# DefaultRui/VLN-VER

Measured on AMD Instinct MI355X. Metric: viewpoints/sec (multi-view->voxel fwd+bwd), vocc.py config, higher is better.
Workload: dtype bf16

## Files before the change

scratch/lattice_mfma_shape_ab.py:

```python
import argparse
import importlib
import json
import os
import shutil
import statistics
import sys
import tempfile

import torch

ROOT = os.path.dirname(os.path.dirname(os.path.abspath(__file__)))
sys.path.insert(0, ROOT)
hip = importlib.import_module('vln-ver_amd.hipops')
ups = importlib.import_module('vln-ver_amd.dense_heads.upsample')


def load(path):
    hip._lib, hip.LIB_PATH = None, os.path.abspath(path)
    return hip.lib()


def timed(f, n=5):
    f()
    torch.cuda.synchronize()
    a, b = torch.cuda.Event(enable_timing=True), torch.cuda.Event(enable_timing=True)
    a.record()
    for _ in range(n):
        f()
    b.record()
    torch.cuda.synchronize()
    return a.elapsed_time(b) / n


def main():
    ap = argparse.ArgumentParser()
    ap.add_argument('arms', nargs='+', help='name=path; the first is the parent')
    ap.add_argument('--reps', type=int, default=5)
    ap.add_argument('--out', default=None)
    args = ap.parse_args()
    arms = [a.split('=', 1) for a in args.arms]
    tmp = tempfile.mkdtemp()
    arms.append(['parent_copy', shutil.copy(arms[0][1], os.path.join(tmp, 'libver_hip_parent_copy.so'))])
    handles = [(name, load(path)) for name, path in arms]
    out = open(args.out, 'a') if args.out else None

    def emit(rec):
        line = json.dumps(rec)
        print(line, flush=True)
        if out:
            out.write(line + '\n')
            out.flush()

    B, DEV, C, N, layout, hc = 192, 'cuda', 768, 1536, 3, 30
    plan = ups._layer_plan_z4(C, torch.device(DEV))[0]
    m = B * 2 * hc * hc
    e = torch.randn(4, B, 2, hc // 2, hc // 2, 2, C, device=DEV).bfloat16()
    table, _ = ups._const_rows_z4(C, hc, hc, torch.device(DEV), torch.bfloat16)
    g = torch.randn(m, N, device=DEV).bfloat16()
    cls = [(ups._class_segments_z4(c, C), plan[c][1] - plan[c][0]) for c in ups._CLASSES]
    ws = [torch.randn(k, N, device=DEV).bfloat16() for _, k in cls]
    dws = [torch.empty(k, N, dtype=torch.bfloat16, device=DEV) for _, k in cls]
    y = torch.empty(m, N, dtype=torch.bfloat16, device=DEV)
    flops = 2.0 * m * N * sum(k for _, k in cls)

    def forward():
        for (segs, _), w in zip(cls, ws):
            hip.gemm_nn_taps(e, layout, (hc, hc), segs, w, const_rows=table, out=y)

    def wgrad():
        for (segs, _), dw in zip(cls, dws):
            hip.wgrad_tn_segments(e, layout, (hc, hc), segs, g, out=dw, const_rows=table)

    for fam, f in (('gemm_nn_segments', forward), ('wgrad_tn_segments', wgrad)):
        samples = {name: [] for name, _ in handles}
        for _ in range(args.reps):
            for name, h in handles:
                hip._lib = h
                samples[name].append(timed(f))
        med = {k: statistics.median(v) for k, v in samples.items()}
        spread = abs(med[arms[0][0]] - med['parent_copy'])
        for name, _ in handles:
            emit(dict(kind='microbench', family=fam, operands='N(0,1)', arm=name, M=m, K=sum(k for _, k in cls), N=N,
                      ms=[round(x, 4) for x in samples[name]], ms_median=round(med[name], 4), tflops=round(flops / med[name] / 1e9, 1)))
        for name, _ in handles[1:-1]:
            gain = med[arms[0][0]] - med[name]
            emit(dict(kind='verdict', family=fam, operands='N(0,1)', arm=name, parent_ms=round(med[arms[0][0]], 4), new_ms=round(med[name], 4),
                      parent_aa_spread_ms=round(spread, 4), gain_ms=round(gain, 4), speedup=round(med[arms[0][0]] / med[name], 4),
                      clears_twice_the_spread=bool(gain > 2 * spread)))
    shutil.rmtree(tmp, ignore_errors=True)


if __name__ == '__main__':
    main()
```

vln-ver_amd/csrc/ver_gemm.hip:

```cpp
#include "ver_common.h"

namespace {
typedef __bf16 bf16x8 __attribute__((ext_vector_type(8)));
typedef float f32x16 __attribute__((ext_vector_type(16)));
typedef int i32x2 __attribute__((ext_vector_type(2)));
typedef int i32x4 __attribute__((ext_vector_type(4)));
typedef __attribute__((address_space(3))) void lds_void;

constexpr int kTile = 256;
constexpr int kStageBytes = 32768;
constexpr int kStages = 4;
constexpr int kLdsBytes = kStages * kStageBytes;

template <int OFF>
__device__ __forceinline__ i32x2 tr_read(int addr) {
    i32x2 v;
    asm volatile("ds_read_b64_tr_b16 %0, %1 offset:%2" : "=v"(v) : "v"(addr), "n"(OFF) : "memory");
    return v;
}
template <int OFF>
__device__ __forceinline__ i32x4 row_read(int addr) {
    i32x4 v;
    asm volatile("ds_read_b128 %0, %1 offset:%2" : "=v"(v) : "v"(addr), "n"(OFF) : "memory");
    return v;
}
__device__ __forceinline__ bf16x8 frag(i32x2 lo, i32x2 hi) {
    return __builtin_bit_cast(bf16x8, (i32x4)__builtin_shufflevector(lo, hi, 0, 1, 2, 3));
}

struct TapArgs {
    const __bf16* lattice;
    long lattice_bytes;
    int B, H, W, C, ntaps, P;
    const float* rowpos;
    const __bf16* cst;
    long cst_bytes;
    int CW, ncst;
    signed char kind[64], dz[64], dy[64], dx[64];
    signed char pl[64];
    long plane_elems;
};

struct GemmArgs {
    const __bf16* A;
    const __bf16* W;
    const float* bias;
    __bf16* C;
    long lda, ldw, ldc, M;
    int K, N, tiles_n, T, per_xcd;
    int S, Kc;
    float* ws;
    TapArgs t;
};

struct GemmLane {
    int offA0, offA1;
    int offB0, offB1;
    int voA, voW;
    int stepW;
    int stepA16;
    int dmaA, dmaW;
};

constexpr int kOutside = (int)0x80000000;
template <int L>
__device__ __forceinline__ int cell_off(const TapArgs& t, int b, int zl, int y, int x, int dz) {
    if ((unsigned)y >= (unsigned)t.H || (unsigned)x >= (unsigned)t.W || b < 0) return kOutside;
    const int j = dz >> 1;
    int v;
    if (L == 0)
        v = ((b * 4 + zl + dz) * t.H + y) * t.W + x;
    else if (L == 2)
        v = ((((b * 2 + zl) * t.H + y) * t.W + x) << 1) + j;
    else
        v = (((((((y & 1) << 1 | (x & 1)) * t.B + b) * 2 + zl) * (t.H >> 1) + (y >> 1)) * (t.W >> 1) + (x >> 1)) << 1) + j;
    return v * t.C * 2;
}

struct TapLane {
    int b1, zl1, y1, x1, b2, zl2, y2, x2;
    int pos1, pos2;
    int vo1, vo2;
    int chunk;
    int tap, ch;
    int seglen, is_cst;
};

template <int L>
__device__ __forceinline__ void tap_offsets(const TapArgs& t, TapLane& tl, __amdgpu_buffer_rsrc_t& ra) {
    if (t.plane_elems && tl.tap < t.ntaps && !t.kind[tl.tap])
        ra = __builtin_amdgcn_make_buffer_rsrc((void*)(t.lattice + (long)t.pl[tl.tap] * t.plane_elems), 0,
                                               (int)max(0L, min(t.lattice_bytes, 0x7FFFFFFFL)), 0x00020000);
    tl.is_cst = 0;
    tl.seglen = 2 * t.C;
    if (tl.tap < t.ntaps) {
        const int dz = t.dz[tl.tap], dy = t.dy[tl.tap], dx = t.dx[tl.tap];
        if (t.kind[tl.tap]) {
            tl.is_cst = 1;
            tl.seglen = 2 * t.CW;
            tl.vo1 = tl.b1 < 0 ? kOutside : (tl.pos1 * t.ncst + dz) * t.CW * 2 + tl.chunk;
            tl.vo2 = tl.b2 < 0 ? kOutside : (tl.pos2 * t.ncst + dz) * t.CW * 2 + tl.chunk;
        } else {
            const int o1 = cell_off<L>(t, tl.b1, tl.zl1, tl.y1 + dy, tl.x1 + dx, dz);
            const int o2 = cell_off<L>(t, tl.b2, tl.zl2, tl.y2 + dy, tl.x2 + dx, dz);
            tl.vo1 = o1 == kOutside ? kOutside : o1 + tl.chunk;
            tl.vo2 = o2 == kOutside ? kOutside : o2 + tl.chunk;
        }
    } else {
        tl.vo1 = tl.vo2 = kOutside;
    }
}

template <int IMPL>
__device__ __forceinline__ void request_a(char* dst, const GemmLane& c, __amdgpu_buffer_rsrc_t& ra, __amdgpu_buffer_rsrc_t rcst,
                                          int& soA, const TapArgs& t, TapLane& tl) {
    if constexpr (IMPL < 0) {
        __builtin_amdgcn_raw_ptr_buffer_load_lds(ra, (lds_void*)dst, 16, c.voA, soA, 0, 0);
        __builtin_amdgcn_raw_ptr_buffer_load_lds(ra, (lds_void*)(dst + 1024), 16, c.voA, soA + c.stepA16, 0, 0);
        soA += 64;
    } else {
        const int ch = __builtin_amdgcn_readfirstlane(tl.ch);
        if (__builtin_amdgcn_readfirstlane(tl.is_cst)) {
            __builtin_amdgcn_raw_ptr_buffer_load_lds(rcst, (lds_void*)dst, 16, tl.vo1, ch, 0, 0);
            __builtin_amdgcn_raw_ptr_buffer_load_lds(rcst, (lds_void*)(dst + 1024), 16, tl.vo2, ch, 0, 0);
        } else {
            __builtin_amdgcn_raw_ptr_buffer_load_lds(ra, (lds_void*)dst, 16, tl.vo1, ch, 0, 0);
            __builtin_amdgcn_raw_ptr_buffer_load_lds(ra, (lds_void*)(dst + 1024), 16, tl.vo2, ch, 0, 0);
        }
        tl.ch = ch + 64;
        if (tl.ch == __builtin_amdgcn_readfirstlane(tl.seglen)) {
            tl.ch = 0;
            tl.tap = __builtin_amdgcn_readfirstlane(tl.tap) + 1;
            tap_offsets<IMPL>(t, tl, ra);
        }
    }
}


template <int ST, int IMPL>
__device__ __forceinline__ void phase(char* lds, f32x16 (&acc)[4][2], const GemmLane& c, __amdgpu_buffer_rsrc_t& ra,
                                      __amdgpu_buffer_rsrc_t rw, int& soA, int& soW, const TapArgs& t, TapLane& tl,
                                      __amdgpu_buffer_rsrc_t rcst) {
    constexpr int SB = (ST & 1) * kStageBytes;
    constexpr int UP = ST >= 2 ? 65536 : 0;
    const int a0 = c.offA0 + UP, a1 = c.offA1 + UP, b0 = c.offB0 + UP, b1 = c.offB1 + UP;
    i32x4 av[2][4];
    i32x2 bl[2][2], bh[2][2];
    av[0][0] = row_read<SB>(a0);
    av[0][1] = row_read<SB + 2048>(a0);
    bl[0][0] = tr_read<SB + 16384>(b0);
    bh[0][0] = tr_read<SB + 16384 + 512>(b0);
    bl[0][1] = tr_read<SB + 16384>(b1);
    bh[0][1] = tr_read<SB + 16384 + 512>(b1);
    av[0][2] = row_read<SB + 4096>(a0);
    av[0][3] = row_read<SB + 6144>(a0);
    av[1][0] = row_read<SB>(a1);
    av[1][1] = row_read<SB + 2048>(a1);
    bl[1][0] = tr_read<SB + 24576>(b0);
    bh[1][0] = tr_read<SB + 24576 + 512>(b0);
    bl[1][1] = tr_read<SB + 24576>(b1);
    bh[1][1] = tr_read<SB + 24576 + 512>(b1);
    av[1][2] = row_read<SB + 4096>(a1);
    av[1][3] = row_read<SB + 6144>(a1);
    constexpr int DS = ((ST + 2) % kStages) * kStageBytes;
    request_a<IMPL>(lds + DS + c.dmaA, c, ra, rcst, soA, t, tl);
    __builtin_amdgcn_raw_ptr_buffer_load_lds(rw, (lds_void*)(lds + DS + 16384 + c.dmaW), 16, c.voW, soW, 0, 0);
    __builtin_amdgcn_raw_ptr_buffer_load_lds(rw, (lds_void*)(lds + DS + 24576 + c.dmaW), 16, c.voW, soW + c.stepW, 0, 0);
    soW += 2 * c.stepW;
    asm volatile("s_waitcnt vmcnt(4)" ::: "memory");
    __builtin_amdgcn_s_barrier();
    asm volatile("s_waitcnt lgkmcnt(0)"
                 : "+v"(av[0][0]), "+v"(av[0][1]), "+v"(av[0][2]), "+v"(av[0][3]), "+v"(av[1][0]), "+v"(av[1][1]), "+v"(av[1][2]),
                   "+v"(av[1][3]), "+v"(bl[0][0]), "+v"(bh[0][0]), "+v"(bl[0][1]), "+v"(bh[0][1]), "+v"(bl[1][0]), "+v"(bh[1][0]),
                   "+v"(bl[1][1]), "+v"(bh[1][1])
                 :
                 : "memory");
    bf16x8 a[2][4], b[2][2];
#pragma unroll
    for (int u = 0; u < 2; ++u) {
#pragma unroll
        for (int i = 0; i < 4; ++i) a[u][i] = __builtin_bit_cast(bf16x8, av[u][i]);
        b[u][0] = frag(bl[u][0], bh[u][0]);
        b[u][1] = frag(bl[u][1], bh[u][1]);
    }
    __builtin_amdgcn_sched_barrier(0);
    __builtin_amdgcn_s_setprio(1);
#pragma unroll
    for (int u = 0; u < 2; ++u)
#pragma unroll
        for (int it = 0; it < 4; ++it)
#pragma unroll
            for (int jt = 0; jt < 2; ++jt)
                acc[it][jt] = __builtin_amdgcn_mfma_f32_32x32x16_bf16(a[u][it], b[u][jt], acc[it][jt], 0, 0, 0);
    __builtin_amdgcn_s_setprio(0);
    __builtin_amdgcn_sched_barrier(0);
    __builtin_amdgcn_s_barrier();
}

template <int IMPL>
__global__ __launch_bounds__(512) void k_gemm_nn(GemmArgs p) {
    extern __shared__ __attribute__((aligned(1024))) char lds[];
    const int tid = threadIdx.x, lane = tid & 63;
    const int wave = __builtin_amdgcn_readfirstlane(tid >> 6);
    const int wr = wave >> 2, wc = wave & 3;
    const int item = (int)(blockIdx.x & 7) * p.per_xcd + (int)(blockIdx.x >> 3);
    if ((int)(blockIdx.x >> 3) >= p.per_xcd || item >= p.T * p.S) return;
    const int split = item / p.T, tile = item - split * p.T;
    const int mt = tile / p.tiles_n, nt = tile - mt * p.tiles_n;
    const long row0 = (long)mt * kTile;
    const int k0 = split * p.Kc, klen = min(p.Kc, p.K - k0);
    const int nphase = klen / 32;

    const __bf16* ab = IMPL < 0 ? p.A + row0 * p.lda + k0 : p.t.lattice;
    const long abytes = IMPL < 0 ? ((p.M - row0 - 1) * p.lda + klen) * 2 : p.t.lattice_bytes;
    __amdgpu_buffer_rsrc_t ra = __builtin_amdgcn_make_buffer_rsrc((void*)ab, 0, (int)max(0L, min(abytes, 0xFFFFFFFFL)), 0x00020000);
    const __amdgpu_buffer_rsrc_t rcst = __builtin_amdgcn_make_buffer_rsrc((void*)(IMPL < 0 ? ab : p.t.cst), 0,
                                                                          (int)(IMPL < 0 ? 0L : max(0L, min(p.t.cst_bytes, 0x7FFFFFFFL))), 0x00020000);
    const __bf16* wb = p.W + (long)k0 * p.ldw + (long)nt * kTile;
    const long wbytes = ((long)(klen - 1) * p.ldw + p.N - (long)nt * kTile) * 2;
    const __amdgpu_buffer_rsrc_t rw = __builtin_amdgcn_make_buffer_rsrc((void*)wb, 0, (int)max(0L, min(wbytes, 0xFFFFFFFFL)), 0x00020000);
    GemmLane c;
    {
        const int prow = 32 * wave + (lane >> 2);
        const int pch = (lane & 3) ^ ((prow >> 2) & 3);
        c.voA = (int)(prow * p.lda * 2) + pch * 16;
        c.dmaA = wave * 2048;
        c.stepA16 = (int)(16 * p.lda * 2);
        const int wrow = lane >> 3, wch = (lane & 7) ^ (((wrow >> 1) & 1) << 2);
        c.voW = (int)(((8 * (wave >> 2) + wrow) * p.ldw + 64 * (wave & 3)) * 2) + wch * 16;
        c.stepW = (int)(16 * p.ldw * 2);
        c.dmaW = wave * 1024;
    }
    {
        const int lbase = (int)(uintptr_t)(__attribute__((address_space(3))) char*)lds;
        const int i = lane & 31, sw = (i >> 2) & 3;
        c.offA0 = lbase + (128 * wr + i) * 64 + (((lane >> 5) ^ sw) << 4);
        c.offA1 = c.offA0 ^ 32;
        const int q = lane >> 4, cl = lane & 15;
        const int lowch = (2 * (q & 1) + ((cl & 3) >> 1)) ^ (((cl >> 3) & 1) << 2);
        c.offB0 = lbase + ((q >> 1) * 32 + (cl >> 2)) * 128 + lowch * 16 + (cl & 1) * 8 + wc * 1024;
        c.offB1 = c.offB0 ^ 64;
    }
    TapLane tl = {};
    if constexpr (IMPL >= 0) {
        const int prow = 32 * wave + (lane >> 2);
        const int hw = p.t.H * p.t.W;
        auto decode = [&](long r, int& b, int& zl, int& y, int& x) {
            if (r >= p.M) {
                b = -1, zl = y = x = 0;
                return;
            }
            b = (int)(r / p.t.P);
            const int pos = (int)(r - (long)b * p.t.P);
            zl = pos / hw;
            const int rem = pos - zl * hw;
            y = rem / p.t.W;
            x = rem - y * p.t.W;
        };
        decode(row0 + prow, tl.b1, tl.zl1, tl.y1, tl.x1);
        decode(row0 + prow + 16, tl.b2, tl.zl2, tl.y2, tl.x2);
        tl.pos1 = (tl.zl1 * p.t.H + tl.y1) * p.t.W + tl.x1;
        tl.pos2 = (tl.zl2 * p.t.H + tl.y2) * p.t.W + tl.x2;
        tl.chunk = ((lane & 3) ^ ((prow >> 2) & 3)) * 16;
        tl.tap = 0, tl.ch = 0;
        tap_offsets<IMPL>(p.t, tl, ra);
    }
    f32x16 acc[4][2];
#pragma unroll
    for (int it = 0; it < 4; ++it)
#pragma unroll
        for (int jt = 0; jt < 2; ++jt)
#pragma unroll
            for (int r = 0; r < 16; ++r) acc[it][jt][r] = 0.0f;

    int soA = 0, soW = 0;
#pragma unroll
    for (int s = 0; s < 2; ++s) {
        request_a<IMPL>(lds + s * kStageBytes + c.dmaA, c, ra, rcst, soA, p.t, tl);
        __builtin_amdgcn_raw_ptr_buffer_load_lds(rw, (lds_void*)(lds + s * kStageBytes + 16384 + c.dmaW), 16, c.voW, soW, 0, 0);
        __builtin_amdgcn_raw_ptr_buffer_load_lds(rw, (lds_void*)(lds + s * kStageBytes + 24576 + c.dmaW), 16, c.voW, soW + c.stepW, 0, 0);
        soW += 2 * c.stepW;
    }
    asm volatile("s_waitcnt vmcnt(4)" ::: "memory");
    __builtin_amdgcn_s_barrier();
    if (wr == 1) __builtin_amdgcn_s_barrier();

    int s = 0;
    for (; s + kStages <= nphase; s += kStages) {
        phase<0, IMPL>(lds, acc, c, ra, rw, soA, soW, p.t, tl, rcst);
        phase<1, IMPL>(lds, acc, c, ra, rw, soA, soW, p.t, tl, rcst);
        phase<2, IMPL>(lds, acc, c, ra, rw, soA, soW, p.t, tl, rcst);
        phase<3, IMPL>(lds, acc, c, ra, rw, soA, soW, p.t, tl, rcst);
    }
    const int rem = nphase - s;
    if (rem > 0) phase<0, IMPL>(lds, acc, c, ra, rw, soA, soW, p.t, tl, rcst);
    if (rem > 1) phase<1, IMPL>(lds, acc, c, ra, rw, soA, soW, p.t, tl, rcst);
    if (rem > 2) phase<2, IMPL>(lds, acc, c, ra, rw, soA, soW, p.t, tl, rcst);
    if (wr == 0) __builtin_amdgcn_s_barrier();
    asm volatile("s_waitcnt vmcnt(0)" ::: "memory");

    if (p.S > 1) {
        float* out = p.ws + (long)split * p.M * p.N;
        const long i0 = row0 + 128 * wr + 4 * (lane >> 5);
        const int j0 = nt * kTile + 64 * wc + (lane & 31);
#pragma unroll
        for (int it = 0; it < 4; ++it)
#pragma unroll
            for (int jt = 0; jt < 2; ++jt) {
                const int j = j0 + 32 * jt;
#pragma unroll
                for (int r = 0; r < 16; ++r) {
                    const long i = i0 + 32 * it + (r & 3) + 8 * (r >> 2);
                    if (i < p.M && j < p.N) out[i * p.N + j] = acc[it][jt][r];
                }
            }
        return;
    }
    __bf16* cb = p.C + row0 * p.ldc + (long)nt * kTile;
    const long cbytes = ((p.M - row0 - 1) * p.ldc + p.N - (long)nt * kTile) * 2;
    const __amdgpu_buffer_rsrc_t rc = __builtin_amdgcn_make_buffer_rsrc((void*)cb, 0, (int)max(0L, min(cbytes, 0xFFFFFFFFL)), 0x00020000);
    const int ldc2 = (int)(p.ldc * 2);
    const int vbase = (128 * wr + 4 * (lane >> 5)) * ldc2 + (64 * wc + (lane & 31)) * 2;
    const bool haspos = IMPL >= 0 && p.t.rowpos != nullptr;
    const int pos0 = haspos ? (int)((row0 + 128 * wr + 4 * (lane >> 5)) % p.t.P) : 0;
#pragma unroll
    for (int jt = 0; jt < 2; ++jt) {
        const int j = nt * kTile + 64 * wc + 32 * jt + (lane & 31);
        const float bj = (p.bias && j < p.N) ? p.bias[j] : 0.0f;
        const int vo = j < p.N ? vbase + 64 * jt : -2;
#pragma unroll
        for (int it = 0; it < 4; ++it) {
            float add[16];
#pragma unroll
            for (int r = 0; r < 16; ++r) {
                add[r] = bj;
                if (haspos) {
                    int pp = pos0 + 32 * it + (r & 3) + 8 * (r >> 2);
                    while (pp >= p.t.P) pp -= p.t.P;
                    const long row = row0 + 128 * wr + 4 * (lane >> 5) + 32 * it + (r & 3) + 8 * (r >> 2);
                    if (j < p.N && row < p.M) add[r] += p.t.rowpos[(long)pp * p.N + j];
                }
            }
#pragma unroll
            for (int r = 0; r < 16; ++r) {
                const __bf16 v = (__bf16)(acc[it][jt][r] + add[r]);
                __builtin_amdgcn_raw_buffer_store_b16(__builtin_bit_cast(short, v), rc, vo, (32 * it + (r & 3) + 8 * (r >> 2)) * ldc2, 0);
            }
        }
    }
}
__global__ __launch_bounds__(256) void k_gemm_reduce(const float* __restrict__ ws, const float* __restrict__ bias,
                                                     __bf16* __restrict__ c, long ldc, int S, long M, int N) {
    const long n4 = M * N / 4;
    const long stride = M * N;
    for (long e = blockIdx.x * 256L + threadIdx.x; e < n4; e += (long)gridDim.x * 256) {
        float4 acc = *reinterpret_cast<const float4*>(ws + 4 * e);
        for (int s = 1; s < S; ++s) {
            const float4 v = *reinterpret_cast<const float4*>(ws + s * stride + 4 * e);
            acc.x += v.x, acc.y += v.y, acc.z += v.z, acc.w += v.w;
        }
        const long i = (4 * e) / N;
        const int j = (int)(4 * e - i * N);
        if (bias) acc.x += bias[j], acc.y += bias[j + 1], acc.z += bias[j + 2], acc.w += bias[j + 3];
        typedef __bf16 bf16x4 __attribute__((ext_vector_type(4)));
        bf16x4 v;
        v.x = (__bf16)acc.x, v.y = (__bf16)acc.y, v.z = (__bf16)acc.z, v.w = (__bf16)acc.w;
        *reinterpret_cast<bf16x4*>(c + i * ldc + j) = v;
    }
}

int pick_k_splits(long M, int K, int N) {
    const long tiles = ((M + kTile - 1) / kTile) * ((N + kTile - 1) / kTile);
    if (tiles >= 96 || K < 2048 || N % 4) return 1;
    int s = (int)((224 + tiles - 1) / tiles);
    if (s > K / 512) s = K / 512;
    if (s > 64) s = 64;
    return s < 2 ? 1 : s;
}
}
// ... 100 lines not shown
                    i, -1 - taps[3 * i], cst ? ncst : 0);
        K += is_cst ? cw : C;
    }
    VER_REQUIRE(lbytes < 0x7FFFFFFFL, VER_EUNSUPPORTED, "ver_gemm_nn_taps: the source lattice (%ld bytes) exceeds the 2-GiB range of the tap offsets", lbytes);
    VER_REQUIRE(ldw >= N && ldc >= N && ldw % 8 == 0 && ((uintptr_t)w & 15) == 0 && ((uintptr_t)lattice & 15) == 0, VER_EUNSUPPORTED,
                "ver_gemm_nn_taps: w must be 16-byte aligned with a row pitch that is a multiple of 8 elements");
    VER_REQUIRE(K * ldw * 2 < 0xFFFFFFFFL && 256L * ldc * 2 < 0x7FFFFFFFL && K < 0x7FFFFFFFL, VER_EUNSUPPORTED,
                "ver_gemm_nn_taps: a tile's operand range exceeds the 32-bit offsets");
    GemmArgs p;
    p.A = nullptr;
    p.W = (const __bf16*)w;
    p.bias = bias;
    p.C = (__bf16*)c;
    p.lda = 0;
    p.ldw = ldw;
    p.ldc = ldc;
    p.M = M;
    p.K = (int)K;
    p.N = N;
    p.tiles_n = (N + kTile - 1) / kTile;
    p.T = (int)((M + kTile - 1) / kTile) * p.tiles_n;
    p.Kc = (int)K;
    p.S = 1;
    p.ws = nullptr;
    p.per_xcd = (p.T + 7) / 8;
    p.t = TapArgs{};
    p.t.lattice = (const __bf16*)lattice;
    p.t.lattice_bytes = lbytes;
    p.t.B = B, p.t.H = H, p.t.W = W, p.t.C = C, p.t.ntaps = ntaps, p.t.P = 2 * H * W;
    p.t.rowpos = rowpos;
    VER_REQUIRE((plane_elems == 0) == (tap_plane == nullptr) && plane_elems >= 0 && (plane_elems == 0 || (nplanes > 0 && nplanes <= 64 &&
                plane_elems % 8 == 0)), VER_EINVAL, "ver_gemm_nn_planes: plane_elems, nplanes and tap_plane come together");
    p.t.plane_elems = plane_elems;
    for (int i = 0; i < ntaps; ++i) {
        VER_REQUIRE(!tap_plane || (tap_plane[i] >= 0 && tap_plane[i] < nplanes), VER_EINVAL, "ver_gemm_nn_planes: tap %d reads plane %d of %d", i,
                    tap_plane ? tap_plane[i] : 0, nplanes);
        p.t.pl[i] = (signed char)(tap_plane ? tap_plane[i] : 0);
    }
    p.t.cst = (const __bf16*)cst;
    p.t.cst_bytes = cst ? (long)2 * H * W * ncst * cw * 2 : 0;
    p.t.CW = cw, p.t.ncst = ncst;
    for (int i = 0; i < ntaps; ++i) {
        const int dz = taps[3 * i], dy = taps[3 * i + 1], dx = taps[3 * i + 2];
        if (dz < 0) {
            p.t.kind[i] = 1, p.t.dz[i] = (signed char)(-1 - dz), p.t.dy[i] = p.t.dx[i] = 0;
            continue;
        }
        VER_REQUIRE((dz == 0 || dz == 2) && dy >= -64 && dy <= 64 && dx >= -64 && dx <= 64, VER_EINVAL,
                    "ver_gemm_nn_taps: tap %d = (%d, %d, %d): dz must be 0 or 2", i, dz, dy, dx);
        p.t.kind[i] = 0, p.t.dz[i] = (signed char)dz, p.t.dy[i] = (signed char)dy, p.t.dx[i] = (signed char)dx;
    }
    hipError_t e = hipSuccess;
#define VER_GEMM_TAPS(L)                                                                                                  \
    do {                                                                                                                  \
        e = hipFuncSetAttribute((const void*)k_gemm_nn<L>, hipFuncAttributeMaxDynamicSharedMemorySize, kLdsBytes);       \
        if (e == hipSuccess) hipLaunchKernelGGL(k_gemm_nn<L>, dim3((unsigned)(8 * p.per_xcd)), dim3(512), kLdsBytes, st, p); \
    } while (0)
    if (layout == 0) VER_GEMM_TAPS(0);
    else if (layout == 2) VER_GEMM_TAPS(2);
    else VER_GEMM_TAPS(3);
#undef VER_GEMM_TAPS
    if (e != hipSuccess) return ver_fail(VER_ELAUNCH, "ver_gemm_nn_taps: LDS attribute: %s", hipGetErrorString(e));
    return ver_check_launch("ver_gemm_nn_taps");
}
```

Before: 722.6.

## Switch GEMM to 16x16 MFMA tiles and pack tap descriptors into scalar kernarg loads

Parameterises the GEMM wave tile by MFMA shape and selects 16x16x? MFMA (8x4 fragments of f32x4) instead of 32x32 (4x2 of f32x16), with matching LDS swizzles and epilogue row mapping. Tap metadata is packed into one 32-bit descriptor per tap and fetched with s_load from the kernarg segment, prefetching the next tap's descriptor so tap transitions avoid per-lane byte-array lookups and readfirstlane calls. The constant-row path now just swaps the buffer resource. This risks more LDS read traffic per FLOP with smaller MFMA tiles and relies on manual lgkmcnt waits for correctness.

```diff
diff --git a/scratch/lattice_gemm_launch.py b/scratch/lattice_gemm_launch.py
--- /dev/null
+++ b/scratch/lattice_gemm_launch.py
@@ -0,0 +1,58 @@
+import collections
+import importlib
+import json
+import os
+import sqlite3
+import sys
+
+ROOT = os.path.dirname(os.path.dirname(os.path.abspath(__file__)))
+sys.path.insert(0, ROOT)
+
+
+def report(path, arm):
+    cur = sqlite3.connect(path).cursor()
+    rows = cur.execute("select kernel_name, counter_name, sum(value), count(distinct dispatch_id) from counters_collection "
+                       "group by kernel_name, counter_name").fetchall()
+    out = collections.defaultdict(dict)
+    for k, c, v, n in rows:
+        if 'k_gemm_nn' in k:
+            name = k.replace('(anonymous namespace)::', '').replace('void ', '').split('(')[0]
+            out[name][c] = round(v / n, 1)
+            out[name]['dispatches'] = n
+    for d in out.values():
+        if 'GRBM_GUI_ACTIVE' in d and 'SQ_VALU_MFMA_BUSY_CYCLES' in d:
+            d['mfma_util'] = round(d['SQ_VALU_MFMA_BUSY_CYCLES'] / (d['GRBM_GUI_ACTIVE'] / 8.0 * 1024.0), 4)
+    print(json.dumps(dict(kind='counters', arm=arm, per_dispatch=out)))
+
+
+def main():
+    import torch
+    hip = importlib.import_module('vln-ver_amd.hipops')
+    ups = importlib.import_module('vln-ver_amd.dense_heads.upsample')
+    lattice_plan = importlib.import_module('vln-ver_amd.dense_heads.lattice_plan')
+    B = int(sys.argv[1]) if len(sys.argv) > 1 else 192
+    calls = int(sys.argv[2]) if len(sys.argv) > 2 else 2
+    dev, C, N, hc = torch.device('cuda'), 768, 1536, 30
+    torch.manual_seed(0)
+    plan = ups._layer_plan_z4(C, dev)[0]
+    table, _ = ups._const_rows_z4(C, hc, hc, dev, torch.bfloat16)
+    cls = [(ups._class_segments_z4(c, C), plan[c][1] - plan[c][0]) for c in ups._CLASSES]
+    _, dtaps, dplanes, nb = lattice_plan._dgrad_plan('lat', C, dev)
+    e = torch.randn(4, B, 2, hc // 2, hc // 2, 2, C, device=dev).bfloat16()
+    ws = [torch.randn(k, N, device=dev).bfloat16() for _, k in cls]
+    gp = torch.randn(4, B, 2, hc, hc, 2, C, device=dev).bfloat16()
+    wd = torch.randn(nb * 2 * C, 2 * C, device=dev).bfloat16()
+    m = B * 2 * hc * hc
+    y = torch.empty(m, N, dtype=torch.bfloat16, device=dev)
+    for _ in range(calls):
+        for (segs, _), w in zip(cls, ws):
+            hip.gemm_nn_taps(e, 3, (hc, hc), segs, w, const_rows=table, out=y)
+        hip.gemm_nn_taps(gp, 2, (hc, hc), dtaps, wd, planes=dplanes, out=y)
+    torch.cuda.synchronize()
+
+
+if __name__ == '__main__':
+    if len(sys.argv) > 1 and sys.argv[1] == 'report':
+        report(sys.argv[2], sys.argv[3])
+    else:
+        main()
diff --git a/scratch/lattice_mfma_shape_ab.py b/scratch/lattice_mfma_shape_ab.py
--- a/scratch/lattice_mfma_shape_ab.py
+++ b/scratch/lattice_mfma_shape_ab.py
@@ -13,6 +13,7 @@
 sys.path.insert(0, ROOT)
 hip = importlib.import_module('vln-ver_amd.hipops')
 ups = importlib.import_module('vln-ver_amd.dense_heads.upsample')
+lattice_plan = importlib.import_module('vln-ver_amd.dense_heads.lattice_plan')
 
 
 def load(path):
@@ -37,6 +38,8 @@
     ap.add_argument('arms', nargs='+', help='name=path; the first is the parent')
     ap.add_argument('--reps', type=int, default=5)
     ap.add_argument('--out', default=None)
+    ap.add_argument('--families', default='gemm_nn_segments,gemm_nn_planes,wgrad_tn_segments')
+    ap.add_argument('--viewpoints', type=int, default=192)
     args = ap.parse_args()
     arms = [a.split('=', 1) for a in args.arms]
     tmp = tempfile.mkdtemp()
@@ -51,42 +54,78 @@
             out.write(line + '\n')
             out.flush()
 
-    B, DEV, C, N, layout, hc = 192, 'cuda', 768, 1536, 3, 30
+    B, DEV, C, N, layout, hc = args.viewpoints, 'cuda', 768, 1536, 3, 30
     plan = ups._layer_plan_z4(C, torch.device(DEV))[0]
     m = B * 2 * hc * hc
-    e = torch.randn(4, B, 2, hc // 2, hc // 2, 2, C, device=DEV).bfloat16()
     table, _ = ups._const_rows_z4(C, hc, hc, torch.device(DEV), torch.bfloat16)
-    g = torch.randn(m, N, device=DEV).bfloat16()
     cls = [(ups._class_segments_z4(c, C), plan[c][1] - plan[c][0]) for c in ups._CLASSES]
-    ws = [torch.randn(k, N, device=DEV).bfloat16() for _, k in cls]
-    dws = [torch.empty(k, N, dtype=torch.bfloat16, device=DEV) for _, k in cls]
-    y = torch.empty(m, N, dtype=torch.bfloat16, device=DEV)
-    flops = 2.0 * m * N * sum(k for _, k in cls)
+    _, dtaps, dplanes, nb = lattice_plan._dgrad_plan('lat', C, torch.device(DEV))
+    kd = nb * 2 * C
+    makes = (('N(0,1)', lambda *s: torch.randn(*s, device=DEV).bfloat16()),
+             ('constant 0.5', lambda *s: torch.full(s, 0.5, device=DEV, dtype=torch.bfloat16)),
+             ('zeros', lambda *s: torch.zeros(*s, device=DEV, dtype=torch.bfloat16)))
+    for dist, make in makes:
+        e = make(4, B, 2, hc // 2, hc // 2, 2, C)
+        g = make(m, N)
+        ws = [make(k, N) for _, k in cls]
+        dws = [torch.empty(k, N, dtype=torch.bfloat16, device=DEV) for _, k in cls]
+        y = torch.empty(m, N, dtype=torch.bfloat16, device=DEV)
+        gp = make(4, B, 2, hc, hc, 2, C)
+        wd = make(kd, 2 * C)
+        de = torch.empty(m, 2 * C, dtype=torch.bfloat16, device=DEV)
+        kf = sum(k for _, k in cls)
 
-    def forward():
-        for (segs, _), w in zip(cls, ws):
-            hip.gemm_nn_taps(e, layout, (hc, hc), segs, w, const_rows=table, out=y)
+        def forward():
+            for (segs, _), w in zip(cls, ws):
+                hip.gemm_nn_taps(e, layout, (hc, hc), segs, w, const_rows=table, out=y)
 
-    def wgrad():
-        for (segs, _), dw in zip(cls, dws):
-            hip.wgrad_tn_segments(e, layout, (hc, hc), segs, g, out=dw, const_rows=table)
+        def wgrad():
+            for (segs, _), dw in zip(cls, dws):
+                hip.wgrad_tn_segments(e, layout, (hc, hc), segs, g, out=dw, const_rows=table)
 
-    for fam, f in (('gemm_nn_segments', forward), ('wgrad_tn_segments', wgrad)):
-        samples = {name: [] for name, _ in handles}
-        for _ in range(args.reps):
+        def planes():
+            hip.gemm_nn_taps(gp, 2, (hc, hc), dtaps, wd, planes=dplanes, out=de)
+
+        if dist == 'N(0,1)':
+            want = {}
             for name, h in handles:
                 hip._lib = h
-                samples[name].append(timed(f))
-        med = {k: statistics.median(v) for k, v in samples.items()}
-        spread = abs(med[arms[0][0]] - med['parent_copy'])
-        for name, _ in handles:
-            emit(dict(kind='microbench', family=fam, operands='N(0,1)', arm=name, M=m, K=sum(k for _, k in cls), N=N,
-                      ms=[round(x, 4) for x in samples[name]], ms_median=round(med[name], 4), tflops=round(flops / med[name] / 1e9, 1)))
-        for name, _ in handles[1:-1]:
-            gain = med[arms[0][0]] - med[name]
-            emit(dict(kind='verdict', family=fam, operands='N(0,1)', arm=name, parent_ms=round(med[arms[0][0]], 4), new_ms=round(med[name], 4),
-                      parent_aa_spread_ms=round(spread, 4), gain_ms=round(gain, 4), speedup=round(med[arms[0][0]] / med[name], 4),
-                      clears_twice_the_spread=bool(gain > 2 * spread)))
+                res = [hip.gemm_nn_taps(e, layout, (hc, hc), segs, w, const_rows=table) for (segs, _), w in zip(cls, ws)]
+                planes()
+                res.append(de.clone())
+                torch.cuda.synchronize()
+                if not want:
+                    want = res
+                else:
+                    emit(dict(kind='bit_identity', arm=name, against=arms[0][0], operands=dist,
+                              gemm_nn_segments=all(torch.equal(a, b) for a, b in zip(res[:-1], want[:-1])),
+                              gemm_nn_planes=bool(torch.equal(res[-1], want[-1]))))
+                del res
+            del want
+            torch.cuda.empty_cache()
+
+        fams = (('gemm_nn_segments', forward, kf, 2.0 * m * N * kf), ('gemm_nn_planes', planes, kd, 2.0 * m * kd * 2 * C),
+                ('wgrad_tn_segments', wgrad, kf, 2.0 * m * N * kf))
+        for fam, f, kk, flops in fams:
+            if fam not in args.families.split(','):
+                continue
+            samples = {name: [] for name, _ in handles}
+            for _ in range(args.reps):
+                for name, h in handles:
+                    hip._lib = h
+                    samples[name].append(timed(f))
+            med = {k: statistics.median(v) for k, v in samples.items()}
+            spread = abs(med[arms[0][0]] - med['parent_copy'])
+            for name, _ in handles:
+                emit(dict(kind='microbench', family=fam, operands=dist, arm=name, M=m, K=kk, N=N,
+                          ms=[round(x, 4) for x in samples[name]], ms_median=round(med[name], 4), tflops=round(flops / med[name] / 1e9, 1)))
+            for name, _ in handles[1:-1]:
+                gain = med[arms[0][0]] - med[name]
+                emit(dict(kind='verdict', family=fam, operands=dist, arm=name, parent_ms=round(med[arms[0][0]], 4), new_ms=round(med[name], 4),
+                          parent_aa_spread_ms=round(spread, 4), gain_ms=round(gain, 4), speedup=round(med[arms[0][0]] / med[name], 4),
+                          clears_twice_the_spread=bool(gain > 2 * spread)))
+        del e, g, ws, dws, y, gp, wd, de
+        torch.cuda.empty_cache()
     shutil.rmtree(tmp, ignore_errors=True)
 
 
diff --git a/vln-ver_amd/csrc/ver_gemm.hip b/vln-ver_amd/csrc/ver_gemm.hip
--- a/vln-ver_amd/csrc/ver_gemm.hip
+++ b/vln-ver_amd/csrc/ver_gemm.hip
@@ -3,6 +3,7 @@
 namespace {
 typedef __bf16 bf16x8 __attribute__((ext_vector_type(8)));
 typedef float f32x16 __attribute__((ext_vector_type(16)));
+typedef float f32x4 __attribute__((ext_vector_type(4)));
 typedef int i32x2 __attribute__((ext_vector_type(2)));
 typedef int i32x4 __attribute__((ext_vector_type(4)));
 typedef __attribute__((address_space(3))) void lds_void;
@@ -11,6 +12,30 @@
 constexpr int kStageBytes = 32768;
 constexpr int kStages = 4;
 constexpr int kLdsBytes = kStages * kStageBytes;
+
+constexpr int kShape = 16;
+template <int SH>
+struct Shape {
+    typedef f32x16 acc_t;
+    static constexpr int NI = 4, NJ = 2, NR = 16, TW = 32;
+    static __device__ __forceinline__ int reg_row(int r) { return (r & 3) + 8 * (r >> 2); }
+    static __device__ __forceinline__ int lane_row(int lane) { return 4 * (lane >> 5); }
+    static __device__ __forceinline__ int swz_a(int row) { return (row >> 2) & 3; }
+    static __device__ __forceinline__ int swz_w(int row, int rowhalf) { return ((row >> 1) & 1) << 2; }
+};
+template <>
+struct Shape<16> {
+    typedef f32x4 acc_t;
+    static constexpr int NI = 8, NJ = 4, NR = 4, TW = 16;
+    static __device__ __forceinline__ int reg_row(int r) { return r; }
+    static __device__ __forceinline__ int lane_row(int lane) { return 4 * (lane >> 4); }
+    static __device__ __forceinline__ int swz_a(int row) { return (0 - (row >> 2)) & 3; }
+    static __device__ __forceinline__ int swz_w(int row, int rowhalf) { return (((row >> 1) & 1) << 2) ^ (rowhalf << 1); }
+};
+typedef Shape<kShape> sh;
+static_assert(Shape<32>::NI * Shape<32>::TW == 128 && Shape<32>::NJ * Shape<32>::TW == 64 && Shape<32>::NI * Shape<32>::NJ * Shape<32>::NR == 128 &&
+                  Shape<16>::NI * Shape<16>::TW == 128 && Shape<16>::NJ * Shape<16>::TW == 64 && Shape<16>::NI * Shape<16>::NJ * Shape<16>::NR == 128,
+              "a wave tile is 128 x 64 in 128 accumulator registers");
 
 template <int OFF>
 __device__ __forceinline__ i32x2 tr_read(int addr) {
@@ -36,8 +61,7 @@
     const __bf16* cst;
     long cst_bytes;
     int CW, ncst;
-    signed char kind[64], dz[64], dy[64], dx[64];
-    signed char pl[64];
+    unsigned desc[64];
     long plane_elems;
 };
 
@@ -55,7 +79,7 @@
 
 struct GemmLane {
     int offA0, offA1;
-    int offB0, offB1;
+    int offB[4];
     int voA, voW;
     int stepW;
     int stepA16;
@@ -82,68 +106,124 @@
     int pos1, pos2;
     int vo1, vo2;
     int chunk;
+};
+struct TapWave {
     int tap, ch;
-    int seglen, is_cst;
+    int seglen;
+    unsigned next;
+    const __attribute__((address_space(4))) unsigned* tab;
 };
 
+__device__ __forceinline__ unsigned desc_load(const TapWave& ts, int idx) {
+    unsigned v;
+    asm volatile("s_load_dword %0, %1, %2" : "=s"(v) : "s"(ts.tab), "s"(idx * 4) : "memory");
+    return v;
+}
+__device__ __forceinline__ void desc_ready(unsigned& d) { asm volatile("s_waitcnt lgkmcnt(0)" : "+s"(d) : : "memory"); }
+
 template <int L>
-__device__ __forceinline__ void tap_offsets(const TapArgs& t, TapLane& tl, __amdgpu_buffer_rsrc_t& ra) {
-    if (t.plane_elems && tl.tap < t.ntaps && !t.kind[tl.tap])
-        ra = __builtin_amdgcn_make_buffer_rsrc((void*)(t.lattice + (long)t.pl[tl.tap] * t.plane_elems), 0,
+__device__ __forceinline__ void tap_begin(const TapArgs& t, TapLane& tl, TapWave& ts, unsigned d, __amdgpu_buffer_rsrc_t& ra,
+                                          __amdgpu_buffer_rsrc_t rcst) {
+    const bool live = ts.tap < t.ntaps;
+    const bool is_cst = live && (d >> 31) != 0;
+    const int dx = (int)(d << 24) >> 24, dy = (int)(d << 16) >> 24, dz = (int)(d >> 16) & 63, pl = (int)(d >> 22) & 63;
+    int o1 = kOutside, o2 = kOutside, seglen = 2 * t.C;
+    if (is_cst) {
+        seglen = 2 * t.CW;
+        if (tl.b1 >= 0) o1 = (tl.pos1 * t.ncst + dz) * t.CW * 2 + tl.chunk;
+        if (tl.b2 >= 0) o2 = (tl.pos2 * t.ncst + dz) * t.CW * 2 + tl.chunk;
+        ra = rcst;
+    } else if (live) {
+        const int c1 = cell_off<L>(t, tl.b1, tl.zl1, tl.y1 + dy, tl.x1 + dx, dz);
+        const int c2 = cell_off<L>(t, tl.b2, tl.zl2, tl.y2 + dy, tl.x2 + dx, dz);
+        if (c1 != kOutside) o1 = c1 + tl.chunk;
+        if (c2 != kOutside) o2 = c2 + tl.chunk;
+        ra = __builtin_amdgcn_make_buffer_rsrc((void*)(t.lattice + (long)pl * t.plane_elems), 0,
                                                (int)max(0L, min(t.lattice_bytes, 0x7FFFFFFFL)), 0x00020000);
-    tl.is_cst = 0;
-    tl.seglen = 2 * t.C;
-    if (tl.tap < t.ntaps) {
-        const int dz = t.dz[tl.tap], dy = t.dy[tl.tap], dx = t.dx[tl.tap];
-        if (t.kind[tl.tap]) {
-            tl.is_cst = 1;
-            tl.seglen = 2 * t.CW;
-            tl.vo1 = tl.b1 < 0 ? kOutside : (tl.pos1 * t.ncst + dz) * t.CW * 2 + tl.chunk;
-            tl.vo2 = tl.b2 < 0 ? kOutside : (tl.pos2 * t.ncst + dz) * t.CW * 2 + tl.chunk;
-        } else {
-            const int o1 = cell_off<L>(t, tl.b1, tl.zl1, tl.y1 + dy, tl.x1 + dx, dz);
-            const int o2 = cell_off<L>(t, tl.b2, tl.zl2, tl.y2 + dy, tl.x2 + dx, dz);
-            tl.vo1 = o1 == kOutside ? kOutside : o1 + tl.chunk;
-            tl.vo2 = o2 == kOutside ? kOutside : o2 + tl.chunk;
-        }
-    } else {
-        tl.vo1 = tl.vo2 = kOutside;
-    }
-}
-
-template <int IMPL>
+    }
+    ts.seglen = seglen;
+    tl.vo1 = o1;
+    tl.vo2 = o2;
+}
+
+template <int IMPL, bool PRO>
 __device__ __forceinline__ void request_a(char* dst, const GemmLane& c, __amdgpu_buffer_rsrc_t& ra, __amdgpu_buffer_rsrc_t rcst,
-                                          int& soA, const TapArgs& t, TapLane& tl) {
+                                          int& soA, const TapArgs& t, TapLane& tl, TapWave& ts) {
     if constexpr (IMPL < 0) {
         __builtin_amdgcn_raw_ptr_buffer_load_lds(ra, (lds_void*)dst, 16, c.voA, soA, 0, 0);
         __builtin_amdgcn_raw_ptr_buffer_load_lds(ra, (lds_void*)(dst + 1024), 16, c.voA, soA + c.stepA16, 0, 0);
         soA += 64;
     } else {
-        const int ch = __builtin_amdgcn_readfirstlane(tl.ch);
-        if (__builtin_amdgcn_readfirstlane(tl.is_cst)) {
-            __builtin_amdgcn_raw_ptr_buffer_load_lds(rcst, (lds_void*)dst, 16, tl.vo1, ch, 0, 0);
-            __builtin_amdgcn_raw_ptr_buffer_load_lds(rcst, (lds_void*)(dst + 1024), 16, tl.vo2, ch, 0, 0);
-        } else {
-            __builtin_amdgcn_raw_ptr_buffer_load_lds(ra, (lds_void*)dst, 16, tl.vo1, ch, 0, 0);
-            __builtin_amdgcn_raw_ptr_buffer_load_lds(ra, (lds_void*)(dst + 1024), 16, tl.vo2, ch, 0, 0);
+        __builtin_amdgcn_raw_ptr_buffer_load_lds(ra, (lds_void*)dst, 16, tl.vo1, ts.ch, 0, 0);
+        __builtin_amdgcn_raw_ptr_buffer_load_lds(ra, (lds_void*)(dst + 1024), 16, tl.vo2, ts.ch, 0, 0);
+        ts.ch += 64;
+        if (ts.ch == ts.seglen) {
+            ts.ch = 0;
+            ts.tap += 1;
+            const unsigned d = ts.next;
+            ts.next = desc_load(ts, min(ts.tap + 1, t.ntaps - 1));
+            if constexpr (PRO) desc_ready(ts.next);
+            tap_begin<IMPL>(t, tl, ts, d, ra, rcst);
         }
-        tl.ch = ch + 64;
-        if (tl.ch == __builtin_amdgcn_readfirstlane(tl.seglen)) {
-            tl.ch = 0;
-            tl.tap = __builtin_amdgcn_readfirstlane(tl.tap) + 1;
-            tap_offsets<IMPL>(t, tl, ra);
-        }
-    }
-}
-
+    }
+}
 
 template <int ST, int IMPL>
-__device__ __forceinline__ void phase(char* lds, f32x16 (&acc)[4][2], const GemmLane& c, __amdgpu_buffer_rsrc_t& ra,
-                                      __amdgpu_buffer_rsrc_t rw, int& soA, int& soW, const TapArgs& t, TapLane& tl,
+__device__ __forceinline__ void phase(char* lds, f32x4 (&acc)[8][4], const GemmLane& c, __amdgpu_buffer_rsrc_t& ra,
+                                      __amdgpu_buffer_rsrc_t rw, int& soA, int& soW, const TapArgs& t, TapLane& tl, TapWave& ts,
                                       __amdgpu_buffer_rsrc_t rcst) {
     constexpr int SB = (ST & 1) * kStageBytes;
     constexpr int UP = ST >= 2 ? 65536 : 0;
-    const int a0 = c.offA0 + UP, a1 = c.offA1 + UP, b0 = c.offB0 + UP, b1 = c.offB1 + UP;
+    const int a0 = c.offA0 + UP;
+    i32x4 av[8];
+    i32x2 bl[4], bh[4];
+    av[0] = row_read<SB>(a0);
+    av[1] = row_read<SB + 1024>(a0);
+#pragma unroll
+    for (int q = 0; q < 4; ++q) {
+        const int b = c.offB[q] + UP;
+        bl[q] = tr_read<SB + 16384>(b);
+        bh[q] = tr_read<SB + 16384 + 512>(b);
+        if (q == 0) av[2] = row_read<SB + 2048>(a0), av[3] = row_read<SB + 3072>(a0);
+        if (q == 1) av[4] = row_read<SB + 4096>(a0), av[5] = row_read<SB + 5120>(a0);
+        if (q == 2) av[6] = row_read<SB + 6144>(a0), av[7] = row_read<SB + 7168>(a0);
+    }
+    constexpr int DS = ((ST + 2) % kStages) * kStageBytes;
+    request_a<IMPL, false>(lds + DS + c.dmaA, c, ra, rcst, soA, t, tl, ts);
+    __builtin_amdgcn_raw_ptr_buffer_load_lds(rw, (lds_void*)(lds + DS + 16384 + c.dmaW), 16, c.voW, soW, 0, 0);
+    __builtin_amdgcn_raw_ptr_buffer_load_lds(rw, (lds_void*)(lds + DS + 24576 + c.dmaW), 16, c.voW, soW + c.stepW, 0, 0);
+    soW += 2 * c.stepW;
+    asm volatile("s_waitcnt vmcnt(4)" ::: "memory");
+    __builtin_amdgcn_s_barrier();
+    asm volatile("s_waitcnt lgkmcnt(0)"
+                 : "+v"(av[0]), "+v"(av[1]), "+v"(av[2]), "+v"(av[3]), "+v"(av[4]), "+v"(av[5]), "+v"(av[6]), "+v"(av[7]), "+v"(bl[0]),
+                   "+v"(bh[0]), "+v"(bl[1]), "+v"(bh[1]), "+v"(bl[2]), "+v"(bh[2]), "+v"(bl[3]), "+v"(bh[3])
+                 :
+                 : "memory");
+    if constexpr (IMPL >= 0) asm volatile("" : "+s"(ts.next));
+    bf16x8 a[8], b[4];
+#pragma unroll
+    for (int i = 0; i < 8; ++i) a[i] = __builtin_bit_cast(bf16x8, av[i]);
+#pragma unroll
+    for (int j = 0; j < 4; ++j) b[j] = frag(bl[j], bh[j]);
+    __builtin_amdgcn_sched_barrier(0);
+    __builtin_amdgcn_s_setprio(1);
+#pragma unroll
+    for (int it = 0; it < 8; ++it)
+#pragma unroll
+        for (int jt = 0; jt < 4; ++jt) acc[it][jt] = __builtin_amdgcn_mfma_f32_16x16x32_bf16(a[it], b[jt], acc[it][jt], 0, 0, 0);
+    __builtin_amdgcn_s_setprio(0);
+    __builtin_amdgcn_sched_barrier(0);
+    __builtin_amdgcn_s_barrier();
+}
+
+template <int ST, int IMPL>
+__device__ __forceinline__ void phase(char* lds, f32x16 (&acc)[4][2], const GemmLane& c, __amdgpu_buffer_rsrc_t& ra,
+                                      __amdgpu_buffer_rsrc_t rw, int& soA, int& soW, const TapArgs& t, TapLane& tl, TapWave& ts,
+                                      __amdgpu_buffer_rsrc_t rcst) {
+    constexpr int SB = (ST & 1) * kStageBytes;
+    constexpr int UP = ST >= 2 ? 65536 : 0;
+    const int a0 = c.offA0 + UP, a1 = c.offA1 + UP, b0 = c.offB[0] + UP, b1 = c.offB[1] + UP;
     i32x4 av[2][4];
     i32x2 bl[2][2], bh[2][2];
     av[0][0] = row_read<SB>(a0);
@@ -163,7 +243,7 @@
     av[1][2] = row_read<SB + 4096>(a1);
     av[1][3] = row_read<SB + 6144>(a1);
     constexpr int DS = ((ST + 2) % kStages) * kStageBytes;
-    request_a<IMPL>(lds + DS + c.dmaA, c, ra, rcst, soA, t, tl);
+    request_a<IMPL, false>(lds + DS + c.dmaA, c, ra, rcst, soA, t, tl, ts);
     __builtin_amdgcn_raw_ptr_buffer_load_lds(rw, (lds_void*)(lds + DS + 16384 + c.dmaW), 16, c.voW, soW, 0, 0);
     __builtin_amdgcn_raw_ptr_buffer_load_lds(rw, (lds_void*)(lds + DS + 24576 + c.dmaW), 16, c.voW, soW + c.stepW, 0, 0);
     soW += 2 * c.stepW;
@@ -175,6 +255,7 @@
                    "+v"(bl[1][1]), "+v"(bh[1][1])
                  :
                  : "memory");
+    if constexpr (IMPL >= 0) asm volatile("" : "+s"(ts.next));
     bf16x8 a[2][4], b[2][2];
 #pragma unroll
     for (int u = 0; u < 2; ++u) {
@@ -222,26 +303,39 @@
     GemmLane c;
     {
         const int prow = 32 * wave + (lane >> 2);
-        const int pch = (lane & 3) ^ ((prow >> 2) & 3);
+        const int pch = (lane & 3) ^ sh::swz_a(prow & 15);
         c.voA = (int)(prow * p.lda * 2) + pch * 16;
         c.dmaA = wave * 2048;
         c.stepA16 = (int)(16 * p.lda * 2);
-        const int wrow = lane >> 3, wch = (lane & 7) ^ (((wrow >> 1) & 1) << 2);
+        const int wrow = lane >> 3, wch = (lane & 7) ^ sh::swz_w(wrow, wave >> 2);
         c.voW = (int)(((8 * (wave >> 2) + wrow) * p.ldw + 64 * (wave & 3)) * 2) + wch * 16;
         c.stepW = (int)(16 * p.ldw * 2);
         c.dmaW = wave * 1024;
     }
     {
         const int lbase = (int)(uintptr_t)(__attribute__((address_space(3))) char*)lds;
-        const int i = lane & 31, sw = (i >> 2) & 3;
-        c.offA0 = lbase + (128 * wr + i) * 64 + (((lane >> 5) ^ sw) << 4);
-        c.offA1 = c.offA0 ^ 32;
-        const int q = lane >> 4, cl = lane & 15;
-        const int lowch = (2 * (q & 1) + ((cl & 3) >> 1)) ^ (((cl >> 3) & 1) << 2);
-        c.offB0 = lbase + ((q >> 1) * 32 + (cl >> 2)) * 128 + lowch * 16 + (cl & 1) * 8 + wc * 1024;
-        c.offB1 = c.offB0 ^ 64;
+        if constexpr (kShape == 32) {
+            const int i = lane & 31;
+            c.offA0 = lbase + (128 * wr + i) * 64 + (((lane >> 5) ^ sh::swz_a(i & 15)) << 4);
+            c.offA1 = c.offA0 ^ 32;
+            const int q = lane >> 4, cl = lane & 15;
+            const int lowch = (2 * (q & 1) + ((cl & 3) >> 1)) ^ sh::swz_w(cl >> 2, q >> 1);
+            c.offB[0] = lbase + ((q >> 1) * 32 + (cl >> 2)) * 128 + lowch * 16 + (cl & 1) * 8 + wc * 1024;
+            c.offB[1] = c.offB[0] ^ 64;
+            c.offB[2] = c.offB[3] = 0;
+        } else {
+            const int i = lane & 15, g = lane >> 4;
+            c.offA0 = lbase + (128 * wr + i) * 64 + ((g ^ sh::swz_a(i)) << 4);
+            c.offA1 = 0;
+#pragma unroll
+            for (int q = 0; q < 4; ++q) {
+                const int ch = (2 * q + ((i & 3) >> 1)) ^ sh::swz_w(i >> 2, g & 1);
+                c.offB[q] = lbase + (g >> 1) * 8192 + (g & 1) * 4096 + (i >> 2) * 128 + ch * 16 + (i & 1) * 8 + wc * 1024;
+            }
+        }
     }
     TapLane tl = {};
+    TapWave ts = {};
     if constexpr (IMPL >= 0) {
         const int prow = 32 * wave + (lane >> 2);
         const int hw = p.t.H * p.t.W;
@@ -261,22 +355,27 @@
         decode(row0 + prow + 16, tl.b2, tl.zl2, tl.y2, tl.x2);
         tl.pos1 = (tl.zl1 * p.t.H + tl.y1) * p.t.W + tl.x1;
         tl.pos2 = (tl.zl2 * p.t.H + tl.y2) * p.t.W + tl.x2;
-        tl.chunk = ((lane & 3) ^ ((prow >> 2) & 3)) * 16;
-        tl.tap = 0, tl.ch = 0;
-        tap_offsets<IMPL>(p.t, tl, ra);
-    }
-    f32x16 acc[4][2];
-#pragma unroll
-    for (int it = 0; it < 4; ++it)
-#pragma unroll
-        for (int jt = 0; jt < 2; ++jt)
-#pragma unroll
-            for (int r = 0; r < 16; ++r) acc[it][jt][r] = 0.0f;
+        tl.chunk = ((lane & 3) ^ sh::swz_a(prow & 15)) * 16;
+        ts.tab = (const __attribute__((address_space(4))) unsigned*)((const __attribute__((address_space(4))) char*)
+                     __builtin_amdgcn_kernarg_segment_ptr() + offsetof(GemmArgs, t) + offsetof(TapArgs, desc));
+        unsigned d = desc_load(ts, 0);
+        desc_ready(d);
+        ts.next = desc_load(ts, min(1, p.t.ntaps - 1));
+        tap_begin<IMPL>(p.t, tl, ts, d, ra, rcst);
+        desc_ready(ts.next);
+    }
+    sh::acc_t acc[sh::NI][sh::NJ];
+#pragma unroll
+    for (int it = 0; it < sh::NI; ++it)
+#pragma unroll
+        for (int jt = 0; jt < sh::NJ; ++jt)
+#pragma unroll
+            for (int r = 0; r < sh::NR; ++r) acc[it][jt][r] = 0.0f;
 
     int soA = 0, soW = 0;
 #pragma unroll
     for (int s = 0; s < 2; ++s) {
-        request_a<IMPL>(lds + s * kStageBytes + c.dmaA, c, ra, rcst, soA, p.t, tl);
+        request_a<IMPL, true>(lds + s * kStageBytes + c.dmaA, c, ra, rcst, soA, p.t, tl, ts);
         __builtin_amdgcn_raw_ptr_buffer_load_lds(rw, (lds_void*)(lds + s * kStageBytes + 16384 + c.dmaW), 16, c.voW, soW, 0, 0);
         __builtin_amdgcn_raw_ptr_buffer_load_lds(rw, (lds_void*)(lds + s * kStageBytes + 24576 + c.dmaW), 16, c.voW, soW + c.stepW, 0, 0);
         soW += 2 * c.stepW;
@@ -287,30 +386,30 @@
 
     int s = 0;
     for (; s + kStages <= nphase; s += kStages) {
-        phase<0, IMPL>(lds, acc, c, ra, rw, soA, soW, p.t, tl, rcst);
-        phase<1, IMPL>(lds, acc, c, ra, rw, soA, soW, p.t, tl, rcst);
-        phase<2, IMPL>(lds, acc, c, ra, rw, soA, soW, p.t, tl, rcst);
-        phase<3, IMPL>(lds, acc, c, ra, rw, soA, soW, p.t, tl, rcst);
+        phase<0, IMPL>(lds, acc, c, ra, rw, soA, soW, p.t, tl, ts, rcst);
+        phase<1, IMPL>(lds, acc, c, ra, rw, soA, soW, p.t, tl, ts, rcst);
+        phase<2, IMPL>(lds, acc, c, ra, rw, soA, soW, p.t, tl, ts, rcst);
+        phase<3, IMPL>(lds, acc, c, ra, rw, soA, soW, p.t, tl, ts, rcst);
     }
     const int rem = nphase - s;
-    if (rem > 0) phase<0, IMPL>(lds, acc, c, ra, rw, soA, soW, p.t, tl, rcst);
-    if (rem > 1) phase<1, IMPL>(lds, acc, c, ra, rw, soA, soW, p.t, tl, rcst);
-    if (rem > 2) phase<2, IMPL>(lds, acc, c, ra, rw, soA, soW, p.t, tl, rcst);
+    if (rem > 0) phase<0, IMPL>(lds, acc, c, ra, rw, soA, soW, p.t, tl, ts, rcst);
+    if (rem > 1) phase<1, IMPL>(lds, acc, c, ra, rw, soA, soW, p.t, tl, ts, rcst);
+    if (rem > 2) phase<2, IMPL>(lds, acc, c, ra, rw, soA, soW, p.t, tl, ts, rcst);
     if (wr == 0) __builtin_amdgcn_s_barrier();
     asm volatile("s_waitcnt vmcnt(0)" ::: "memory");
 
     if (p.S > 1) {
         float* out = p.ws + (long)split * p.M * p.N;
-        const long i0 = row0 + 128 * wr + 4 * (lane >> 5);
-        const int j0 = nt * kTile + 64 * wc + (lane & 31);
-#pragma unroll
-        for (int it = 0; it < 4; ++it)
-#pragma unroll
-            for (int jt = 0; jt < 2; ++jt) {
-                const int j = j0 + 32 * jt;
-#pragma unroll
-                for (int r = 0; r < 16; ++r) {
-                    const long i = i0 + 32 * it + (r & 3) + 8 * (r >> 2);
+        const long i0 = row0 + 128 * wr + sh::lane_row(lane);
+        const int j0 = nt * kTile + 64 * wc + (lane & (sh::TW - 1));
+#pragma unroll
+        for (int it = 0; it < sh::NI; ++it)
+#pragma unroll
+            for (int jt = 0; jt < sh::NJ; ++jt) {
+                const int j = j0 + sh::TW * jt;
+#pragma unroll
+                for (int r = 0; r < sh::NR; ++r) {
+                    const long i = i0 + sh::TW * it + sh::reg_row(r);
                     if (i < p.M && j < p.N) out[i * p.N + j] = acc[it][jt][r];
                 }
             }
@@ -320,31 +419,31 @@
     const long cbytes = ((p.M - row0 - 1) * p.ldc + p.N - (long)nt * kTile) * 2;
     const __amdgpu_buffer_rsrc_t rc = __builtin_amdgcn_make_buffer_rsrc((void*)cb, 0, (int)max(0L, min(cbytes, 0xFFFFFFFFL)), 0x00020000);
     const int ldc2 = (int)(p.ldc * 2);
-    const int vbase = (128 * wr + 4 * (lane >> 5)) * ldc2 + (64 * wc + (lane & 31)) * 2;
+    const int vbase = (128 * wr + sh::lane_row(lane)) * ldc2 + (64 * wc + (lane & (sh::TW - 1))) * 2;
     const bool haspos = IMPL >= 0 && p.t.rowpos != nullptr;
-    const int pos0 = haspos ? (int)((row0 + 128 * wr + 4 * (lane >> 5)) % p.t.P) : 0;
-#pragma unroll
-    for (int jt = 0; jt < 2; ++jt) {
-        const int j = nt * kTile + 64 * wc + 32 * jt + (lane & 31);
+    const int pos0 = haspos ? (int)((row0 + 128 * wr + sh::lane_row(lane)) % p.t.P) : 0;
+#pragma unroll
+    for (int jt = 0; jt < sh::NJ; ++jt) {
+        const int j = nt * kTile + 64 * wc + sh::TW * jt + (lane & (sh::TW - 1));
         const float bj = (p.bias && j < p.N) ? p.bias[j] : 0.0f;
-        const int vo = j < p.N ? vbase + 64 * jt : -2;
-#pragma unroll
-        for (int it = 0; it < 4; ++it) {
-            float add[16];
-#pragma unroll
-            for (int r = 0; r < 16; ++r) {
+        const int vo = j < p.N ? vbase + 2 * sh::TW * jt : -2;
+#pragma unroll
+        for (int it = 0; it < sh::NI; ++it) {
+            float add[sh::NR];
+#pragma unroll
+            for (int r = 0; r < sh::NR; ++r) {
                 add[r] = bj;
                 if (haspos) {
-                    int pp = pos0 + 32 * it + (r & 3) + 8 * (r >> 2);
+                    int pp = pos0 + sh::TW * it + sh::reg_row(r);
                     while (pp >= p.t.P) pp -= p.t.P;
-                    const long row = row0 + 128 * wr + 4 * (lane >> 5) + 32 * it + (r & 3) + 8 * (r >> 2);
+                    const long row = row0 + 128 * wr + sh::lane_row(lane) + sh::TW * it + sh::reg_row(r);
                     if (j < p.N && row < p.M) add[r] += p.t.rowpos[(long)pp * p.N + j];
                 }
             }
 #pragma unroll
-            for (int r = 0; r < 16; ++r) {
+            for (int r = 0; r < sh::NR; ++r) {
                 const __bf16 v = (__bf16)(acc[it][jt][r] + add[r]);
-                __builtin_amdgcn_raw_buffer_store_b16(__builtin_bit_cast(short, v), rc, vo, (32 * it + (r & 3) + 8 * (r >> 2)) * ldc2, 0);
+                __builtin_amdgcn_raw_buffer_store_b16(__builtin_bit_cast(short, v), rc, vo, (sh::TW * it + sh::reg_row(r)) * ldc2, 0);
             }
         }
     }
@@ -511,23 +610,20 @@
     VER_REQUIRE((plane_elems == 0) == (tap_plane == nullptr) && plane_elems >= 0 && (plane_elems == 0 || (nplanes > 0 && nplanes <= 64 &&
                 plane_elems % 8 == 0)), VER_EINVAL, "ver_gemm_nn_planes: plane_elems, nplanes and tap_plane come together");
     p.t.plane_elems = plane_elems;
-    for (int i = 0; i < ntaps; ++i) {
-        VER_REQUIRE(!tap_plane || (tap_plane[i] >= 0 && tap_plane[i] < nplanes), VER_EINVAL, "ver_gemm_nn_planes: tap %d reads plane %d of %d", i,
-                    tap_plane ? tap_plane[i] : 0, nplanes);
-        p.t.pl[i] = (signed char)(tap_plane ? tap_plane[i] : 0);
-    }
     p.t.cst = (const __bf16*)cst;
     p.t.cst_bytes = cst ? (long)2 * H * W * ncst * cw * 2 : 0;
     p.t.CW = cw, p.t.ncst = ncst;
     for (int i = 0; i < ntaps; ++i) {
+        VER_REQUIRE(!tap_plane || (tap_plane[i] >= 0 && tap_plane[i] < nplanes), VER_EINVAL, "ver_gemm_nn_planes: tap %d reads plane %d of %d", i,
+                    tap_plane ? tap_plane[i] : 0, nplanes);
         const int dz = taps[3 * i], dy = taps[3 * i + 1], dx = taps[3 * i + 2];
         if (dz < 0) {
-            p.t.kind[i] = 1, p.t.dz[i] = (signed char)(-1 - dz), p.t.dy[i] = p.t.dx[i] = 0;
+            p.t.desc[i] = 0x80000000u | (unsigned)(-1 - dz) << 16;
             continue;
         }
         VER_REQUIRE((dz == 0 || dz == 2) && dy >= -64 && dy <= 64 && dx >= -64 && dx <= 64, VER_EINVAL,
                     "ver_gemm_nn_taps: tap %d = (%d, %d, %d): dz must be 0 or 2", i, dz, dy, dx);
-        p.t.kind[i] = 0, p.t.dz[i] = (signed char)dz, p.t.dy[i] = (signed char)dy, p.t.dx[i] = (signed char)dx;
+        p.t.desc[i] = (unsigned)(tap_plane ? tap_plane[i] : 0) << 22 | (unsigned)dz << 16 | (unsigned)(dy & 0xFF) << 8 | (unsigned)(dx & 0xFF);
     }
     hipError_t e = hipSuccess;
 #define VER_GEMM_TAPS(L)                                                                                                  \
```

New measurement: 762.5, median of 6. 1.06x the previous value.
